# mbrymer/quadrotor_landing

Hardware: NVIDIA B200
Metric: EKF filter-steps/s (propagate+update) (higher is better)
Workload: dtype f64

## Files before the change

### quadrotor_landing_b200/csrc/ekf_kernels.cuh

```cuda
#pragma once

#include <type_traits>

#include "ekf_core.cuh"
#include "ekf_synth.cuh"

namespace qekf {

enum : int32_t {
    FLAG_INIT = 1,
    FLAG_READY = 2,
    FLAG_CORRECTED = 4,
    FLAG_ACTIVE = 8
};

constexpr int AUX_DIM = 11;
constexpr int PEND_DIM = 8;

template <typename T> struct DeviceState {
    T *x;
    T *P;
    T *aux;
    double *pend;
    int32_t *flags;
// ... 27 lines not shown
        return ParUS<T>{ (uint32_t)__cvta_generic_to_shared(csm) };
    }
#endif
};
template <typename T> struct ParSel<T, true> {
    using type = ParF<T>;
    static QEKF_FN type make(const Consts<T> &c, const DeviceState<T> &st, int64_t i)
    {
        return type{ c, st.pf + i, st.pf_delay + i, st.ld };
    }
    static QEKF_FN type make_cold(const type &par, const Consts<T> *, const DeviceState<T> &, int64_t, std::false_type) { return par; }
#ifdef __CUDACC__
    static __device__ __forceinline__ ParFS<T> make_cold(const type &, const Consts<T> *csm, const DeviceState<T> &st, int64_t i, std::true_type)
    {
        return ParFS<T>{ (uint32_t)__cvta_generic_to_shared(csm), st.pf + i, st.pf_delay + i, st.ld };
    }
#endif
};

struct StreamView {
    const double *imu;
    const int32_t *tag_step;
    const double *tag_pose;
    const double *tag_stamp;
    const uint8_t *tag_valid;
    const double *tag_sigma;
    int64_t cs, is;
    int64_t M;
    int64_t vs;
    double t_start;
    double update_freq;
};

template <typename T> struct RunArgs {
    DeviceState<T> st;
    StreamView in;
    Consts<T> c;
    int64_t k0, n_steps;
    int32_t m0;
    NoiseSpec ns;
    StatsView stats;
};

#ifdef __CUDA_ARCH__
#define QEKF_COLD __device__ __noinline__
#else
#define QEKF_COLD inline
#endif

template <typename T, bool SYNTH> struct Inputs {
    const double *imu_i, *tag_i;
    int64_t cs;
    const uint8_t *valid_i;
    int64_t vs;
    int64_t gid;
    double bias[6];
    int32_t priv_start;

    QEKF_FN void init(const RunArgs<T> &a, int64_t i) { init(a, i, i); }
    QEKF_FN void init(const RunArgs<T> &a, int64_t i, int64_t id)
    {
        imu_i = a.in.imu + i * a.in.is;
        tag_i = a.in.tag_pose + i * a.in.is;
        cs = a.in.cs;
        valid_i = (!SYNTH && a.in.tag_valid) ? a.in.tag_valid + i : nullptr;
        vs = a.in.vs;
        gid = a.ns.gid0 + id;
        if (SYNTH) {
            true_bias(a.ns, gid, bias);
            priv_start = private_dropout_start(a.ns, gid);
        }
    }
    QEKF_FN void raw_imu(int64_t k, double u[6]) const
    {
#pragma unroll
// ... 144 lines not shown
    T *x = st.x + i;
#pragma unroll
    for (int k = 0; k < 3; ++k) {
        x[(0 + k) * st.ld] = s.r[k];
        x[(3 + k) * st.ld] = s.v[k];
        x[(10 + k) * st.ld] = s.ab[k];
        x[(13 + k) * st.ld] = s.wb[k];
    }
#pragma unroll
    for (int k = 0; k < 4; ++k) x[(6 + k) * st.ld] = s.q[k];
#pragma unroll 8
    for (int e = 0; e < NP; ++e) st.P[e * st.ld + i] = P.el(e);
}

template <typename T, bool BIAS, bool DIRECT, class PS, class PAR>
QEKF_COLD void correction_call(Nominal<T> *sp, PS &P, const T *tag, const PAR par, Observation<T> *obs)
{
    Nominal<T> s = *sp;
    T tg[7];
#pragma unroll
    for (int cc = 0; cc < 7; ++cc) tg[cc] = tag[cc];
    Observation<T> o;
    correction_step<T, BIAS, DIRECT>(s, P, tg, par, o);
    *sp = s;
    *obs = o;
}

struct CtaVote {
    int active, want, fenced, at_fence, lanes;
    bool out_of_patience;
};
constexpr int VOTE_WORDS = 12;

QEKF_FN void cta_vote_init(int *vbuf)
{
#ifdef __CUDA_ARCH__
    if (threadIdx.x < VOTE_WORDS) vbuf[threadIdx.x] = 0;
    __syncthreads();
#else
    (void)vbuf;
#endif
}

QEKF_FN CtaVote cta_vote(int *vbuf, uint32_t iter, bool active, bool want, bool oop, bool fenced, bool at_fence)
{
    CtaVote r;
#ifdef __CUDA_ARCH__
    const unsigned full = 0xffffffffu;
    const unsigned ma = __ballot_sync(full, active), mw = __ballot_sync(full, want), mo = __ballot_sync(full, oop);
    const unsigned mf = __ballot_sync(full, fenced), mt = __ballot_sync(full, at_fence);
    int *v = vbuf + (iter % 3u) * 4;
    if ((threadIdx.x & 31) == 0) {
        atomicAdd(v + 0, __popc(ma) | (__popc(mw) << 16));
        atomicAdd(v + 1, __popc(mf) | (__popc(mt) << 16));
        if (mo) atomicOr(v + 2, 1);
    }
    __syncthreads();
    const int x0 = v[0], x1 = v[1], x2 = v[2];
    if (threadIdx.x == 0) {
        int *z = vbuf + ((iter + 2u) % 3u) * 4;
        z[0] = 0; z[1] = 0; z[2] = 0;
    }
    r.active = x0 & 0xffff; r.want = x0 >> 16; r.fenced = x1 & 0xffff; r.at_fence = x1 >> 16;
    r.out_of_patience = x2 != 0;
    r.lanes = (int)blockDim.x;
#else
    (void)vbuf; (void)iter;
    r.active = active; r.want = want; r.fenced = fenced; r.at_fence = at_fence; r.out_of_patience = oop; r.lanes = 1;
#endif
    return r;
}

struct WarpVote {
    int active, want, fenced, at_fence, lanes;
    bool out_of_patience;
};
QEKF_FN WarpVote warp_vote(bool active, bool want, bool oop, bool fenced, bool at_fence)
{
    WarpVote r;
#ifdef __CUDA_ARCH__
    const unsigned full = 0xffffffffu;
    r.active = __popc(__ballot_sync(full, active));
    r.want = __popc(__ballot_sync(full, want));
    r.fenced = __popc(__ballot_sync(full, fenced));
    r.at_fence = __popc(__ballot_sync(full, at_fence));
    r.out_of_patience = __ballot_sync(full, oop) != 0u;
    r.lanes = 32;
#else
    r.active = active; r.want = want; r.fenced = fenced; r.at_fence = at_fence; r.out_of_patience = oop; r.lanes = 1;
#endif
    return r;
}
QEKF_FN bool cta_any(bool x)
{
#ifdef __CUDA_ARCH__
    return __syncthreads_or(x) != 0;
#else
    return x;
#endif
}

struct SmemInt {
    int32_t *p;
    QEKF_FN operator int32_t() const { return *p; }
    QEKF_FN SmemInt &operator=(int32_t v) { *p = v; return *this; }
    QEKF_FN SmemInt &operator=(const SmemInt &o) { *p = *o.p; return *this; }
    QEKF_FN SmemInt &operator+=(int32_t v) { *p += v; return *this; }
    QEKF_FN SmemInt &operator-=(int32_t v) { *p -= v; return *this; }
    QEKF_FN SmemInt &operator|=(int32_t v) { *p |= v; return *this; }
    QEKF_FN SmemInt &operator&=(int32_t v) { *p &= v; return *this; }
    QEKF_FN SmemInt &operator++() { *p += 1; return *this; }
};
constexpr int MR_SCRATCH_INTS = 18;
constexpr int SR_SCRATCH_INTS = 16;

template <typename T, bool BIAS, bool DIRECT, bool SYNTH, bool PF, class PS, bool CSM = false>
QEKF_FN void run_filter(const RunArgs<T> &a, const int64_t i_in, PS &P, int32_t *scr, const int scr_stride,
                        const bool live = true, int *vbuf = nullptr, const Consts<T> *c_cold = nullptr)
{
    const Consts<T> &c = a.c;
    const int64_t i = live ? i_in : 0;
    const typename ParSel<T, PF>::type par = ParSel<T, PF>::make(a.c, a.st, i);
    const auto par_cold = ParSel<T, PF>::make_cold(par, c_cold, a.st, i, std::integral_constant<bool, CSM>());
    const int32_t k_end = (int32_t)(a.k0 + a.n_steps);
    Nominal<T> s;
    SmemInt flags{ scr + 0 * scr_stride }, upds{ scr + 1 * scr_stride }, n_pred{ scr + 2 * scr_stride };
    SmemInt n_corr{ scr + 3 * scr_stride }, n_iter{ scr + 4 * scr_stride }, m{ scr + 5 * scr_stride };
    SmemInt next_tag_step{ scr + 6 * scr_stride }, pend_m{ scr + 7 * scr_stride }, held{ scr + 8 * scr_stride };
    SmemInt k{ scr + 9 * scr_stride };
    flags = 0; upds = 0; n_pred = 0; n_corr = 0; n_iter = 0;
    T accel[3] = { T(0), T(0), T(0) };
    Inputs<T, SYNTH> in;
    double un[6] = { 0, 0, 0, 0, 0, 0 };
    k = k_end;
    if (live) {
        load_filter<T>(a.st, i, s, P);
        flags = a.st.flags[i];
        upds = a.st.upds[i];
#pragma unroll
        for (int cc = 0; cc < 3; ++cc) accel[cc] = a.st.aux[cc * a.st.ld + i];
        in.init(a, i, a.st.gid_perm ? (int64_t)a.st.gid_perm[i] : i);
        k = (int32_t)a.k0;
        if (SYNTH) {
            float z[6];
            normals6(a.ns, in.gid, STREAM_BIAS, 0u, z);
#pragma unroll
            for (int cc = 0; cc < 6; ++cc) reinterpret_cast<float *>(scr)[(10 + cc) * scr_stride] = z[cc];
        } else {
            in.raw_imu(k, un);
        }
    }
    auto true_bias_now = [&](double b[6]) {
#pragma unroll
        for (int cc = 0; cc < 6; ++cc)
            b[cc] = (double)(cc < 3 ? a.ns.sig_ba : a.ns.sig_bw) * (double)reinterpret_cast<const float *>(scr)[(10 + cc) * scr_stride];
    };

    uint32_t n_sexec = 0, n_cev = 0;
    m = a.m0;
    next_tag_step = (m < a.in.M) ? a.in.tag_step[m] : INT32_MAX;
    pend_m = -1;
    held = 0;
    bool at_fence = false;
    const bool do_stats = SYNTH && a.stats.acc != nullptr;
    const int32_t patience = c.limit_measurement_freq ? (c.upd_per_meas - 1) : 0;
    int32_t next_fence = do_stats ? (int32_t)((a.k0 / a.stats.stride + 1) * a.stats.stride) : INT32_MAX;
    bool predicted = false;

    cta_vote_init(vbuf);
    for (uint32_t iter = 0;; ++iter) {
        bool want = predicted;
        if (k < k_end && !at_fence && !predicted) {
            int32_t kk = k, up = upds, fl = flags, nts = next_tag_step, np_run = 0;
            for (;;) {
                if (kk == nts) {
                    const int32_t mm = m;
                    if (in.valid(a.in, a.ns, mm, kk)) {
                        pend_m = mm;
                        fl |= FLAG_READY;
                        if (!(fl & FLAG_INIT)) {
                            T tag0[7];
                            in.tag(a.in, a.ns, mm, tag0);
                            initialize_state<T, BIAS>(s, P, tag0, par, false);
                            fl |= FLAG_INIT;
                        }
                    }
                    m = mm + 1;
                    nts = (mm + 1 < a.in.M) ? a.in.tag_step[mm + 1] : INT32_MAX;
                }
                const bool init = (fl & FLAG_INIT) != 0;
                const bool gate = init && (fl & FLAG_READY) && (!c.limit_measurement_freq || (up + 1) >= c.upd_per_meas);
                if (init) {
                    T u[6];
                    if (SYNTH) {
                        double raw[6], tb[6], ud[6];
                        in.raw_imu(a.in, kk, raw);
                        true_bias_now(tb);
                        synth_imu(a.ns, in.gid, kk, raw, tb, ud);
#pragma unroll
                        for (int cc = 0; cc < 6; ++cc) u[cc] = (T)ud[cc];
                    } else {
                        in.imu(a.ns, kk, un, u);
                    }
                    prediction_step<T, BIAS>(s, P, u, par, accel);
                    ++np_run;
                }
                if (gate) { want = true; break; }
                if (init) {
                    up += 1;
                    fl = (fl & ~FLAG_CORRECTED) | FLAG_ACTIVE;
                }
                ++kk;
                if (!SYNTH && kk < k_end) in.raw_imu(kk, un);
                if (kk == next_fence) { at_fence = true; break; }
                if (kk >= k_end) break;
            }
            k = kk; upds = up; flags = fl; next_tag_step = nts;
            n_pred += np_run;
            predicted = want;
        }
        const bool active = (k < k_end) && !at_fence;
        const int32_t fl0 = flags;
        const CtaVote v = cta_vote(vbuf, iter, active, want, want && held >= patience, at_fence || k >= k_end, at_fence);
        if (v.active == 0 && v.at_fence == 0) break;
        ++n_iter;
        if (do_stats && v.fenced == v.lanes && v.at_fence != 0) {
            const bool mine = live && at_fence && (fl0 & FLAG_INIT);
            double tb[6] = { 0, 0, 0, 0, 0, 0 };
            if (SYNTH) true_bias_now(tb);
            stats_sample<T, BIAS>(a, i, (int64_t)k - 1, s, P, tb, mine);
            if (mine) ++n_sexec;
            at_fence = false;
            next_fence += a.stats.stride;
        }
        bool serve = true;
        if (v.want != 0) serve = (2 * v.want > v.active) || v.out_of_patience;
        if (want && !serve) ++held;

#if defined(__CUDA_ARCH__) && defined(QEKF_DIAG_EVENTS)
        if (__ballot_sync(0xffffffffu, want && serve) != 0u) ++n_cev;
#endif
        if (want && serve) {
            T tag[7];
            if (pend_m >= 0) {
                in.tag(a.in, a.ns, pend_m, tag);
            } else {
#pragma unroll
                for (int cc = 0; cc < 7; ++cc) tag[cc] = (T)a.st.pend[cc * a.st.ld + i];
            }
            flags &= ~FLAG_READY;
            const bool perform = c.corner_margin_enbl ? corner_gate<T>(tag, c) : true;
            held = 0;
            if (perform) {
                ++n_corr;
                Observation<T> obs;
                correction_step<T, BIAS, DIRECT>(s, P, tag, par, obs);
// ... 559 lines not shown
        advance(&s, k - nh, nh, accel, a.st.ring + i);
        store_filter<T>(a.st, i, s, P);
        hp = (nh > 0) ? nh - 1 : 0;
    }
    a.st.flags[i] = flags;
    a.st.upds[i] = upds;
    a.st.nh[i] = nh; a.st.hpos[i] = hp; a.st.hlen[i] = hlen;
    if (a.st.counts) {
#ifdef __CUDA_ARCH__
        atomicAdd(a.st.counts + 0, (unsigned long long)(uint32_t)(int32_t)n_pred);
        atomicAdd(a.st.counts + 1, (unsigned long long)n_corr);
        if ((i & 31) == 0) atomicAdd(a.st.counts + 2, (unsigned long long)n_iter);
        atomicAdd(a.st.counts + 4, (unsigned long long)n_sexec);
#else
        a.st.counts[0] += (uint32_t)(int32_t)n_pred;
        a.st.counts[1] += n_corr;
#endif
    }
#pragma unroll
    for (int cc = 0; cc < 3; ++cc) a.st.aux[cc * a.st.ld + i] = accel[cc];
}

template <typename T> __device__ __forceinline__ void copy_consts(Consts<T> *dst, const Consts<T> &src)
{
#ifdef __CUDA_ARCH__
    static_assert(sizeof(Consts<T>) % 8 == 0, "Consts is copied in 8-byte words");
    const unsigned long long *s = reinterpret_cast<const unsigned long long *>(&src);
    unsigned long long *d = reinterpret_cast<unsigned long long *>(dst);
    for (unsigned w = threadIdx.x; w < sizeof(Consts<T>) / 8; w += blockDim.x) d[w] = s[w];
#endif
}
constexpr size_t consts_smem_bytes(size_t consts_size) { return (consts_size + 15) / 16 * 16; }

template <typename T, bool BIAS, bool DIRECT, bool SYNTH, bool MR, bool PF, int BLOCK>
__global__ void __launch_bounds__(BLOCK, 1) run_kernel(const __grid_constant__ RunArgs<T> a)
{
    constexpr int N = BIAS ? 15 : 9;
    extern __shared__ __align__(16) unsigned char smem_raw[];
    T *sm = reinterpret_cast<T *>(smem_raw);
    const int64_t slot = (int64_t)blockIdx.x * BLOCK + threadIdx.x;
    const bool live = slot < a.st.n;
    const int64_t i = slot;
    PShared<T, N, BLOCK> P{ sm + threadIdx.x };
#ifdef QEKF_EXP8
    int *vbuf = reinterpret_cast<int *>(sm + (size_t)BLOCK * ((sizeof(T) == 8 && N == 15) ? 105 : N * (N + 1) / 2));
#else
    int *vbuf = reinterpret_cast<int *>(sm + (size_t)BLOCK * (N * (N + 1) / 2));
#endif
    int32_t *scr = vbuf + VOTE_WORDS;
    Consts<T> *csm = reinterpret_cast<Consts<T> *>(scr + (size_t)BLOCK * (MR ? MR_SCRATCH_INTS : SR_SCRATCH_INTS));
#ifndef QEKF_EXP8
    copy_consts(csm, a.c);
#else
    csm = nullptr;
#endif
#ifndef QEKF_EXP8
    if constexpr (MR && SYNTH) {
        if (a.st.hist_synth) run_filter_mrs<T, BIAS, DIRECT, PF, PShared<T, N, BLOCK>, true>(a, i, P, scr + threadIdx.x, BLOCK, live, vbuf, csm);
        else run_filter_mr<T, BIAS, DIRECT, SYNTH, PF, PShared<T, N, BLOCK>, true>(a, i, P, scr + threadIdx.x, BLOCK, live, vbuf, csm);
    } else if constexpr (MR) {
        run_filter_mr<T, BIAS, DIRECT, SYNTH, PF, PShared<T, N, BLOCK>, true>(a, i, P, scr + threadIdx.x, BLOCK, live, vbuf, csm);
    } else {
        run_filter<T, BIAS, DIRECT, SYNTH, PF, PShared<T, N, BLOCK>, true>(a, i, P, scr + threadIdx.x, BLOCK, live, vbuf, csm);
    }
#else
    if (MR) run_filter_mr<T, BIAS, DIRECT, SYNTH, PF>(a, i, P, scr + threadIdx.x, BLOCK, live, vbuf, csm);
    else run_filter<T, BIAS, DIRECT, SYNTH, PF>(a, i, P, scr + threadIdx.x, BLOCK, live, vbuf, csm);
#endif
}

template <typename T, class PS>
QEKF_FN void rebase_history(const DeviceState<T> &st, int64_t i, const Nominal<T> &s, const PS &P)
{
    if (!st.xc) return;
    store_checkpoint<T>(st, i, s, P);
    st.nh[i] = 0;
    st.hlen[i] = 1;
}

template <typename T, bool BIAS, bool PF, class PS>
QEKF_FN void deliver_one(const DeviceState<T> &st, const Consts<T> &c, const double *pose8, int force_init, int reinit_bias,
                         int raise_ready, PS &P, int64_t i)
{
    int32_t flags = st.flags[i];
    if (!force_init) {
#pragma unroll
        for (int cc = 0; cc < PEND_DIM; ++cc) st.pend[cc * st.ld + i] = pose8[cc];
        if (raise_ready) flags |= FLAG_READY;
    }
    if (force_init || (raise_ready && !(flags & FLAG_INIT))) {
        Nominal<T> s;
        load_filter<T>(st, i, s, P);
        T tag[7];
#pragma unroll
        for (int cc = 0; cc < 7; ++cc) tag[cc] = (T)st.pend[cc * st.ld + i];
        const typename ParSel<T, PF>::type par = ParSel<T, PF>::make(c, st, i);
        initialize_state<T, BIAS>(s, P, tag, par, reinit_bias != 0);
        store_filter<T>(st, i, s, P);
        rebase_history<T>(st, i, s, P);
        flags |= FLAG_INIT;
    }
// ... 132 lines not shown
```

### quadrotor_landing_b200/csrc/ekf_synth.cuh

```cuda
#pragma once

#include <cmath>

#include "ekf_core.cuh"

namespace qekf {

struct NoiseSpec {
    uint64_t seed;
    int64_t gid0;
    float sig_a, sig_w;
    float sig_ba, sig_bw;
    float sig_p, sig_th;
    int32_t drop_k0, drop_k1;
    int32_t rdrop_len, rdrop_lo, rdrop_hi;
    int32_t edge_loss;
    double range_ref, range_exp_p, range_exp_th;
};

enum : uint32_t { STREAM_IMU = 0, STREAM_TAG = 2, STREAM_BIAS = 4, STREAM_DROPOUT = 6 };

QEKF_FN uint32_t mulhi32(uint32_t a, uint32_t b)
{
#ifdef __CUDA_ARCH__
// ... 66 lines not shown

QEKF_FN void true_bias(const NoiseSpec &ns, int64_t gid, double b[6])
{
    float z[6];
    normals6(ns, gid, STREAM_BIAS, 0u, z);
#pragma unroll
    for (int i = 0; i < 3; ++i) {
        b[i] = (double)ns.sig_ba * (double)z[i];
        b[3 + i] = (double)ns.sig_bw * (double)z[3 + i];
    }
}

QEKF_FN int32_t private_dropout_start(const NoiseSpec &ns, int64_t gid)
{
    if (ns.rdrop_len <= 0 || ns.rdrop_hi <= ns.rdrop_lo) return INT32_MAX;
    uint32_t w[4];
    philox4x32_10(0u, STREAM_DROPOUT, (uint32_t)(uint64_t)gid, (uint32_t)((uint64_t)gid >> 32), (uint32_t)ns.seed,
                  (uint32_t)(ns.seed >> 32), w);
    const uint32_t span = (uint32_t)(ns.rdrop_hi - ns.rdrop_lo);
    return ns.rdrop_lo + (int32_t)mulhi32(w[0], span);
}

QEKF_FN bool arrival_valid(const NoiseSpec &ns, int32_t step, int32_t priv_start)
{
    if (step >= ns.drop_k0 && step < ns.drop_k1) return false;
    if (priv_start != INT32_MAX && step >= priv_start && step < priv_start + ns.rdrop_len) return false;
    return true;
}

struct ImuSynth {
    uint64_t seed;
    float sig_a, sig_w, sig_ba, sig_bw;
};
QEKF_FN void synth_imu(const ImuSynth &nz, int64_t gid, int64_t k, const double clean[6], const double bias[6], double u[6])
{
    float z[6];
    normals6(nz.seed, gid, STREAM_IMU, (uint32_t)k, z);
#pragma unroll
    for (int i = 0; i < 3; ++i) {
        u[i] = clean[i] + bias[i] + (double)nz.sig_a * (double)z[i];
        u[3 + i] = clean[3 + i] + bias[3 + i] + (double)nz.sig_w * (double)z[3 + i];
    }
}
QEKF_FN void synth_imu(const NoiseSpec &ns, int64_t gid, int64_t k, const double clean[6], const double bias[6], double u[6])
{
    const ImuSynth nz{ ns.seed, ns.sig_a, ns.sig_w, ns.sig_ba, ns.sig_bw };
    synth_imu(nz, gid, k, clean, bias, u);
}

template <typename T> QEKF_FN bool bundle_in_image(const double tag[7], const Consts<T> &c)
{
    double R[9];
    quat_to_rot<double>(tag + 3, R);
    for (int i = 0; i < c.n_tags; ++i) {
        const double hw = (double)c.tag_hw[i], px0 = (double)c.tag_px[i], py0 = (double)c.tag_py[i];
        bool all_in = true;
#pragma unroll
        for (int k = 0; k < 4; ++k) {
            const double cx = ((k == 0 || k == 3) ? hw : -hw) + px0;
            const double cy = ((k < 2) ? hw : -hw) + py0;
            const double p0 = R[0] * cx + R[1] * cy + tag[0];
            const double p1 = R[3] * cx + R[4] * cy + tag[1];
            const double p2 = R[6] * cx + R[7] * cy + tag[2];
            const double iz = 1.0 / p2;
            const double xn = p0 * iz, yn = p1 * iz;
            const double uu = (double)c.Kcam[0] * xn + (double)c.Kcam[1] * yn + (double)c.Kcam[2];
            const double vv = (double)c.Kcam[3] * xn + (double)c.Kcam[4] * yn + (double)c.Kcam[5];
            all_in = all_in && (p2 > 0.0) && (uu > 0.0) && (uu < (double)c.cam_w) && (vv > 0.0) && (vv < (double)c.cam_h);
        }
        if (all_in) return true;
    }
    return false;
}

inline void visibility_mask(const double *tag_pose_clean, int64_t M, const Consts<double> &c, uint8_t *out)
// ... 122 lines not shown
```

### quadrotor_landing_b200/csrc/inst_run.cu

```cuda
#include "launch.hpp"

namespace qekf {

template <typename T, bool BIAS, bool DIRECT, bool SYNTH, bool MR, bool PF>
cudaError_t launch_run(const RunArgs<T> &a, unsigned grid, size_t smem, cudaStream_t stream)
{
    auto kern = run_kernel<T, BIAS, DIRECT, SYNTH, MR, PF, BlockOf<T>::value>;
    cudaError_t e = prep_kernel(kern, smem);
    if (e != cudaSuccess) return e;
    kern<<<grid, BlockOf<T>::value, smem, stream>>>(a);
    return cudaGetLastError();
}

template <typename T, bool BIAS, bool DIRECT, bool MR>
cudaError_t launch_tick(const RunArgs<T> &a, const double *pose8, int tag_mode, double *out, int n_out, cudaStream_t stream)
{
    constexpr int N = BIAS ? 15 : 9;
    auto kern = tick_kernel<T, BIAS, DIRECT, MR>;
    const size_t smem = (size_t)TICK_BLOCK * (N * (N + 1) / 2) * sizeof(T) + VOTE_WORDS * sizeof(int) +
                        (size_t)TICK_BLOCK * (MR ? MR_SCRATCH_INTS : SR_SCRATCH_INTS) * sizeof(int32_t);
    static unsigned prepared = 0;
    int dev = 0;
    cudaGetDevice(&dev);
    if (!(prepared & (1u << (dev & 31)))) {
        cudaError_t e = cudaFuncSetAttribute(kern, cudaFuncAttributeMaxDynamicSharedMemorySize, (int)smem);
        if (e != cudaSuccess) return e;
        prepared |= 1u << (dev & 31);
    }
    const unsigned grid = (unsigned)((a.st.n + TICK_BLOCK - 1) / TICK_BLOCK);
    kern<<<grid, TICK_BLOCK, smem, stream>>>(a, pose8, tag_mode, out, n_out);
    return cudaGetLastError();
}
template cudaError_t launch_tick<Q_T, (Q_BIAS != 0), (Q_DIRECT != 0), (Q_MR != 0)>(const RunArgs<Q_T> &, const double *, int,
                                                                                   double *, int, cudaStream_t);

#define INST(S, PF_)                                                                                                  \
    template cudaError_t launch_run<Q_T, (Q_BIAS != 0), (Q_DIRECT != 0), S, (Q_MR != 0), PF_>(const RunArgs<Q_T> &,    \
                                                                                               unsigned, size_t, cudaStream_t);
INST(false, false)
INST(true, false)
INST(false, true)
INST(true, true)

// ... 2 lines not shown
```

### quadrotor_landing_b200/csrc/launch.hpp

```cpp
#pragma once

#include <cuda_runtime.h>

#include "ekf_kernels.cuh"

namespace qekf {

#ifdef QEKF_EXP8
template <typename T> struct BlockOf { static constexpr int value = (sizeof(T) == 4) ? 384 : 256; };
#else
#ifndef QEKF_FP32_BLOCK
#define QEKF_FP32_BLOCK 384
#endif
template <typename T> struct BlockOf { static constexpr int value = (sizeof(T) == 4) ? QEKF_FP32_BLOCK : 224; };
#endif

template <typename T, bool BIAS, bool DIRECT, bool SYNTH, bool MR, bool PF>
cudaError_t launch_run(const RunArgs<T> &a, unsigned grid, size_t smem, cudaStream_t stream);

template <typename T, bool BIAS, bool PF>
cudaError_t launch_deliver(const DeviceState<T> &st, const Consts<T> &c, const double *pose8, int force_init,
                           int reinit_bias, int raise_ready, unsigned grid, size_t smem, cudaStream_t stream);

template <typename T, bool BIAS, bool DIRECT, bool MR>
cudaError_t launch_tick(const RunArgs<T> &a, const double *pose8, int tag_mode, double *out, int n_out, cudaStream_t stream);

template <typename T, bool BIAS, bool PF>
cudaError_t launch_predict(const DeviceState<T> &st, const Consts<T> &c, const double *u, unsigned grid, size_t smem,
                           cudaStream_t stream);

template <typename T, bool BIAS, bool DIRECT, bool PF>
cudaError_t launch_correct(const DeviceState<T> &st, const Consts<T> &c, const double *tag, unsigned grid, size_t smem,
                           cudaStream_t stream);

template <typename T>
cudaError_t launch_reset(const DeviceState<T> &st, const Consts<T> &c, int nstates, int reset_nominal, cudaStream_t stream);

template <typename T> cudaError_t launch_rebase(const DeviceState<T> &st, int np, cudaStream_t stream);

template <typename T>
cudaError_t launch_dump(const RunArgs<T> &a, int64_t first, int64_t count, int64_t T_ticks, double *imu_out,
                        double *tag_out, uint8_t *valid_out, double *bias_out, cudaStream_t stream);

template <typename W>
cudaError_t launch_permute_rows(W *dst, const W *src, const int32_t *perm, int64_t rows, int64_t ld, int64_t n, bool to_slots,
                                cudaStream_t stream);

template <typename T> cudaError_t launch_fma_peak(T *sink, int iters, unsigned grid, unsigned block, cudaStream_t stream);
// ... 12 lines not shown
```

### quadrotor_landing_b200/csrc/qekf_capi.cu

```cuda
#include "../../include/qekf.h"

#include <cuda_runtime.h>

#include <algorithm>
#include <cmath>
#include <cstdio>
#include <cstdlib>
#include <cstring>
#include <new>
#include <string>
#include <type_traits>
#include <vector>

#include "ekf_params.hpp"
#include "launch.hpp"
#include "launch_coop.hpp"
#include "preset.hpp"
#include "scenario.hpp"

using namespace qekf;

namespace {

thread_local std::string g_err;
// ... 26 lines not shown
    double *pend = nullptr;
    int32_t *flags = nullptr, *upds = nullptr;
    unsigned long long *counts = nullptr;
    void *xc = nullptr, *Pc = nullptr, *ring = nullptr;
    int32_t *nh = nullptr, *hpos = nullptr, *hlen = nullptr;
    int ring_len = 0, dmax = 1;
    std::vector<double> pf_host[5];
    bool pf_overridden[5] = { false, false, false, false, false };
    bool pf_on = false;
    void *pf = nullptr;
    double *pf_delay = nullptr;
    double *d_tick = nullptr;
    double *h_tick = nullptr;
    double *tick_in = nullptr, *tick_in_dev = nullptr;
    double *tick_out = nullptr, *tick_out_dev = nullptr;
    int tick_out_cap = 0;
    int32_t *d_no_steps = nullptr;
    double imu_latched[6] = { 0, 0, 0, 0, 0, 0 };
    void *d_in = nullptr;
    size_t d_in_bytes = 0;
    double *stats_acc = nullptr, *stats_red = nullptr;
    int32_t stats_bins = 0, stats_stride = 0;
    void *d_shared = nullptr;
    size_t d_shared_bytes = 0;
    uint8_t *d_mask = nullptr;
    size_t d_mask_bytes = 0;
    int32_t *d_perm = nullptr;
    void *perm_scratch = nullptr;
    size_t perm_scratch_bytes = 0;
    bool in_slot_order = false;
    uint64_t perm_seed = 0;
    int64_t perm_gid0 = 0;
    int32_t perm_len = 0, perm_lo = 0, perm_hi = 0;
    bool perm_on = true;
    int64_t perm_min_steps = 256;
    bool hist_clean = true, hist_key_valid = false, lazy_mr_on = true, lazy_now = false;
    uint64_t hist_key[6] = { 0, 0, 0, 0, 0, 0 };
    int64_t hist_k_next = 0;
    int64_t launches = 0;
    int lanes_per_filter = 1;
    int coop_groups = COOP_GROUPS_DEFAULT, duo_groups = DUO_GROUPS_DEFAULT;
};

namespace {

template <typename T> DeviceState<T> dstate(const qekf_handle *h)
{
    DeviceState<T> s;
    s.x = (T *)h->x; s.P = (T *)h->P; s.aux = (T *)h->aux; s.pend = h->pend;
    s.flags = h->flags; s.upds = h->upds; s.counts = h->counts; s.ld = h->ld; s.n = h->n;
    s.xc = (T *)h->xc; s.Pc = (T *)h->Pc; s.ring = (T *)h->ring;
    s.nh = h->nh; s.hpos = h->hpos; s.hlen = h->hlen;
    s.ring_len = h->ring_len; s.dmax_m1 = h->dmax - 1;
    s.pf = h->pf_on ? (const T *)h->pf : nullptr;
    s.pf_delay = h->pf_on ? h->pf_delay : nullptr;
    s.perm = nullptr;
    s.gid_perm = nullptr;
    s.hist_synth = 0;
    return s;
}

void hist_touch(qekf_handle *h) { h->hist_clean = false; h->hist_key_valid = false; }
void hist_emptied(qekf_handle *h) { h->hist_clean = true; h->hist_key_valid = false; }

uint64_t fnv1a(const void *data, size_t bytes, uint64_t hsh = 1469598103934665603ULL)
{
    const unsigned char *p = static_cast<const unsigned char *>(data);
    for (size_t i = 0; i < bytes; ++i) { hsh ^= p[i]; hsh *= 1099511628211ULL; }
    return hsh;
}

int block_of(const qekf_handle *h) { return h->precision == QEKF_FP64 ? BlockOf<double>::value : BlockOf<float>::value; }
size_t smem_bytes(const qekf_handle *h)
{
#ifdef QEKF_EXP8
    size_t b = (size_t)block_of(h) * ((h->precision == QEKF_FP64 && h->np == 120) ? 105 : h->np) * h->tsize + VOTE_WORDS * sizeof(int);
#else
    size_t b = (size_t)block_of(h) * h->np * h->tsize + VOTE_WORDS * sizeof(int);
#endif
    b += (size_t)block_of(h) * (h->p.multirate_ekf ? MR_SCRATCH_INTS : SR_SCRATCH_INTS) * sizeof(int32_t);
#ifndef QEKF_EXP8
    b += consts_smem_bytes(h->precision == QEKF_FP64 ? sizeof(Consts<double>) : sizeof(Consts<float>));
#endif
    return b;
}
unsigned grid_of(const qekf_handle *h) { return (unsigned)((h->n + block_of(h) - 1) / block_of(h)); }

#define QEKF_DISPATCH(h, CALL)                                                             \
    do {                                                                                   \
        const bool b__ = (h)->p.est_bias != 0, d__ = (h)->p.direct_orien_method != 0;      \
        if ((h)->precision == QEKF_FP64) {                                                 \
            if (b__ && d__) { CALL(double, true, true); }                                  \
            else if (b__) { CALL(double, true, false); }                                   \
            else if (d__) { CALL(double, false, true); }                                   \
            else { CALL(double, false, false); }                                           \
        } else {                                                                           \
            if (b__ && d__) { CALL(float, true, true); }                                   \
            else if (b__) { CALL(float, true, false); }                                    \
            else if (d__) { CALL(float, false, true); }                                    \
            else { CALL(float, false, false); }                                            \
        }                                                                                  \
    } while (0)

int free_state(qekf_handle *h)
{
    cudaFree(h->x); cudaFree(h->P); cudaFree(h->aux); cudaFree(h->pend);
    cudaFree(h->flags); cudaFree(h->upds); cudaFree(h->d_tick); cudaFree(h->d_in);
    cudaFree(h->stats_acc); cudaFree(h->stats_red); cudaFree(h->d_shared); cudaFree(h->counts);
    cudaFree(h->xc); cudaFree(h->Pc); cudaFree(h->ring); cudaFree(h->nh); cudaFree(h->hpos); cudaFree(h->hlen);
    cudaFree(h->pf); cudaFree(h->pf_delay); cudaFree(h->d_mask); cudaFree(h->d_perm); cudaFree(h->perm_scratch);
    h->d_perm = nullptr; h->perm_len = 0; h->perm_scratch = nullptr; h->perm_scratch_bytes = 0; h->in_slot_order = false;
    h->d_mask = nullptr; h->d_mask_bytes = 0;
    h->xc = h->Pc = h->ring = nullptr; h->nh = h->hpos = h->hlen = nullptr; h->ring_len = 0;
    h->pf = nullptr; h->pf_delay = nullptr; h->pf_on = false;
    for (auto &v : h->pf_host) v.clear();
    h->counts = nullptr;
    h->stats_acc = h->stats_red = nullptr; h->stats_bins = 0; h->d_shared = nullptr; h->d_shared_bytes = 0;
    if (h->h_tick) cudaFreeHost(h->h_tick);
    if (h->tick_in) cudaFreeHost(h->tick_in);
    if (h->tick_out) cudaFreeHost(h->tick_out);
    h->tick_in = h->tick_in_dev = h->tick_out = h->tick_out_dev = nullptr; h->tick_out_cap = 0;
    h->x = h->P = h->aux = nullptr; h->pend = nullptr; h->flags = h->upds = nullptr;
    h->d_tick = nullptr; h->h_tick = nullptr; h->d_in = nullptr; h->d_in_bytes = 0;
    return QEKF_OK;
}

int max_step_delay(const qekf_handle *h)
{
    if (h->p.dynamic_meas_delay) return step_of_delay(h->p.measurement_delay_max, h->p.update_freq);
    int d = step_of_delay(h->p.measurement_delay, h->p.update_freq);
    const std::vector<double> &v = h->pf_host[QEKF_PF_DELAY];
    for (int64_t i = 0; i < (int64_t)v.size() / 2; ++i) {
        const int di = step_of_delay(v[(size_t)i], h->p.update_freq);
        if (di > d) d = di;
    }
    return d;
}

int alloc_history(qekf_handle *h)
{
    if (!h->p.multirate_ekf) return QEKF_OK;
    const size_t ld = (size_t)h->ld;
    const int dmax = max_step_delay(h);
// ... 32 lines not shown
}

int alloc_state(qekf_handle *h)
{
    h->nstates = h->p.est_bias ? 15 : 9;
    h->np = h->nstates * (h->nstates + 1) / 2;
    h->tsize = (h->precision == QEKF_FP64) ? 8 : 4;
    const size_t ld = (size_t)h->ld;
    CUDA_TRY(cudaMalloc(&h->x, 16 * ld * h->tsize));
    CUDA_TRY(cudaMalloc(&h->P, (size_t)h->np * ld * h->tsize));
    CUDA_TRY(cudaMalloc(&h->aux, AUX_DIM * ld * h->tsize));
    CUDA_TRY(cudaMalloc(&h->pend, PEND_DIM * ld * sizeof(double)));
    CUDA_TRY(cudaMalloc(&h->flags, ld * sizeof(int32_t)));
    CUDA_TRY(cudaMalloc(&h->upds, ld * sizeof(int32_t)));
    CUDA_TRY(cudaMalloc(&h->counts, 8 * sizeof(unsigned long long)));
    CUDA_TRY(cudaMemsetAsync(h->counts, 0, 8 * sizeof(unsigned long long), h->stream));
    CUDA_TRY(cudaMalloc(&h->d_tick, 16 * sizeof(double)));
    CUDA_TRY(cudaMallocHost(&h->h_tick, 16 * sizeof(double)));
    CUDA_TRY(cudaMemsetAsync(h->x, 0, 16 * ld * h->tsize, h->stream));
    CUDA_TRY(cudaMemsetAsync(h->P, 0, (size_t)h->np * ld * h->tsize, h->stream));
    CUDA_TRY(cudaMemsetAsync(h->aux, 0, AUX_DIM * ld * h->tsize, h->stream));
    CUDA_TRY(cudaMemsetAsync(h->pend, 0, PEND_DIM * ld * sizeof(double), h->stream));
    CUDA_TRY(cudaMemsetAsync(h->flags, 0, ld * sizeof(int32_t), h->stream));
    CUDA_TRY(cudaMemsetAsync(h->upds, 0, ld * sizeof(int32_t), h->stream));
    return alloc_history(h);
}

int reset_cov(qekf_handle *h, bool reset_nominal)
{
    if (h->precision == QEKF_FP64)
        CUDA_TRY(launch_reset<double>(dstate<double>(h), make_consts<double>(h->p), h->nstates, reset_nominal, h->stream));
    else
        CUDA_TRY(launch_reset<float>(dstate<float>(h), make_consts<float>(h->p), h->nstates, reset_nominal, h->stream));
    return QEKF_OK;
}

int check_params(const qekf_params *p)
{
    if (!p) return fail(QEKF_ERR_BAD_ARG, "params is NULL");
    if (!(p->update_freq > 0) || !(p->measurement_freq > 0)) return fail(QEKF_ERR_BAD_ARG, "rates must be positive");
    if (p->n_tags < 0 || p->n_tags > QEKF_MAX_TAGS) return fail(QEKF_ERR_BAD_ARG, "n_tags out of range");
    if (p->multirate_ekf) {
        if (!(p->measurement_delay_max >= 0) || !(p->measurement_delay >= 0))
            return fail(QEKF_ERR_BAD_ARG, "measurement delays must be non-negative");
        if (step_of_delay(p->dynamic_meas_delay ? p->measurement_delay_max : p->measurement_delay, p->update_freq) > 4096)
            return fail(QEKF_ERR_BAD_ARG, "measurement delay spans more than 4096 ticks");
    }
    return QEKF_OK;
}

template <typename T, bool BIAS, bool DIRECT>
int run_typed(qekf_handle *h, const StreamView &in, int64_t k0, int64_t n_steps, int32_t m0, const NoiseSpec *ns,
              const double *truth)
{
    RunArgs<T> a;
    std::memset(&a, 0, sizeof a);
    a.st = dstate<T>(h);
    a.in = in;
    a.c = make_consts<T>(h->p);
    a.k0 = k0; a.n_steps = n_steps; a.m0 = m0;
    if (ns) {
        a.ns = *ns;
        a.st.gid_perm = h->in_slot_order ? h->d_perm : nullptr;
        a.st.hist_synth = h->lazy_now ? 1 : 0;
        if (h->stats_acc && truth && h->stats_stride > 0) {
            a.stats.acc = h->stats_acc; a.stats.truth = truth;
            a.stats.n_bins = h->stats_bins; a.stats.stride = h->stats_stride;
            a.stats.chi2_lo = BIAS ? 6.262137795043251 : 2.7003894999803584;
            a.stats.chi2_hi = BIAS ? 27.488392863442982 : 19.02276779864163;
        }
    }
    const bool mr = h->p.multirate_ekf != 0, pf = h->pf_on;
    if constexpr (std::is_same<T, double>::value) {
        if (!mr && h->lanes_per_filter == 2) {
            cudaError_t e;
            if (ns) e = pf ? launch_run_duo<BIAS, DIRECT, true, true>(a, h->duo_groups, h->stream)
                           : launch_run_duo<BIAS, DIRECT, true, false>(a, h->duo_groups, h->stream);
            else e = pf ? launch_run_duo<BIAS, DIRECT, false, true>(a, h->duo_groups, h->stream)
                        : launch_run_duo<BIAS, DIRECT, false, false>(a, h->duo_groups, h->stream);
            if (e != cudaSuccess) return fail(QEKF_ERR_CUDA, std::string("two-role replay launch: ") + cudaGetErrorString(e));
            h->launches++;
            return QEKF_OK;
        }
        if (!mr && h->lanes_per_filter == 3) {
            cudaError_t e;
            if (ns) e = pf ? launch_run_coop<BIAS, DIRECT, true, true>(a, h->coop_groups, h->stream)
                           : launch_run_coop<BIAS, DIRECT, true, false>(a, h->coop_groups, h->stream);
            else e = pf ? launch_run_coop<BIAS, DIRECT, false, true>(a, h->coop_groups, h->stream)
                        : launch_run_coop<BIAS, DIRECT, false, false>(a, h->coop_groups, h->stream);
            if (e != cudaSuccess) return fail(QEKF_ERR_CUDA, std::string("cooperative replay launch: ") + cudaGetErrorString(e));
            h->launches++;
            return QEKF_OK;
        }
    }
#define LAUNCH_(S, MR_, PF_) CUDA_TRY((launch_run<T, BIAS, DIRECT, S, MR_, PF_>(a, grid_of(h), smem_bytes(h), h->stream)))
#define LAUNCH_S(S)                                                       \
    do {                                                                  \
        if (mr && pf) LAUNCH_(S, true, true);                             \
        else if (mr) LAUNCH_(S, true, false);                             \
        else if (pf) LAUNCH_(S, false, true);                             \
        else LAUNCH_(S, false, false);                                    \
    } while (0)
    if (ns) LAUNCH_S(true);
    else LAUNCH_S(false);
#undef LAUNCH_S
#undef LAUNCH_
    h->launches++;
    return QEKF_OK;
}

int run_dispatch(qekf_handle *h, const StreamView &in, int64_t k0, int64_t n_steps, int32_t m0,
                 const NoiseSpec *ns = nullptr, const double *truth = nullptr)
{
#define CALL_RUN(T, B, D) return run_typed<T, B, D>(h, in, k0, n_steps, m0, ns, truth)
    QEKF_DISPATCH(h, CALL_RUN);
#undef CALL_RUN
    return QEKF_OK;
}

int fetch_rows(qekf_handle *h, const void *dev, int rows, int64_t first, int64_t count, double *out)
{
    CUDA_TRY(cudaStreamSynchronize(h->stream));
    if (h->precision == QEKF_FP64) {
        CUDA_TRY(cudaMemcpy2D(out, (size_t)count * 8, (const char *)dev + (size_t)first * 8, (size_t)h->ld * 8,
                              (size_t)count * 8, (size_t)rows, cudaMemcpyDeviceToHost));
    } else {
        std::vector<float> tmp((size_t)rows * (size_t)count);
        CUDA_TRY(cudaMemcpy2D(tmp.data(), (size_t)count * 4, (const char *)dev + (size_t)first * 4, (size_t)h->ld * 4,
// ... 1206 lines not shown
```

Before: 8.102 billion.

## Add producer warp that precomputes IMU noise into a per-block shared ring

For fp64 Monte-Carlo single-rate runs, the kernel gains an extra warp that generates Gaussian IMU noise ahead of the filter threads. It writes the noise into a global slab ring claimed per block and publishes progress with release/acquire flags in shared memory. Filter threads spin-wait on those flags, read the precomputed noise, and prefetch the next tick's noise and IMU data. Vote barriers switch to a named barrier that covers only the filter threads. The goal is to take RNG cost off the filter's critical path, at the cost of extra threads, spin-waiting, global-memory ring traffic and slab-claim atomics.

```diff
diff --git a/quadrotor_landing_b200/csrc/ekf_kernels.cuh b/quadrotor_landing_b200/csrc/ekf_kernels.cuh
--- a/quadrotor_landing_b200/csrc/ekf_kernels.cuh
+++ b/quadrotor_landing_b200/csrc/ekf_kernels.cuh
@@ -83,6 +83,14 @@
     double update_freq;
 };
 
+struct NoiseRing {
+    float *slab;
+    int32_t *owner;
+    int32_t n_slabs;
+};
+constexpr int NOISE_RING_TICKS = 16;
+constexpr int NOISE_BATCH = 4;
+
 template <typename T> struct RunArgs {
     DeviceState<T> st;
     StreamView in;
@@ -91,7 +99,17 @@
     int32_t m0;
     NoiseSpec ns;
     StatsView stats;
+    NoiseRing nring;
 };
+
+template <typename T, bool SYNTH, bool MR> QEKF_FN constexpr bool has_noise_producer()
+{
+#ifdef QEKF_EXP8
+    return false;
+#else
+    return sizeof(T) == 8 && SYNTH && !MR;
+#endif
+}
 
 #ifdef __CUDA_ARCH__
 #define QEKF_COLD __device__ __noinline__
@@ -302,16 +320,25 @@
 };
 constexpr int VOTE_WORDS = 12;
 
-QEKF_FN void cta_vote_init(int *vbuf)
+template <int NT> QEKF_FN void filter_sync()
+{
+#ifdef __CUDA_ARCH__
+    if constexpr (NT == 0) __syncthreads();
+    else asm volatile("bar.sync 1, %0;" ::"n"(NT) : "memory");
+#endif
+}
+
+template <int NT = 0> QEKF_FN void cta_vote_init(int *vbuf)
 {
 #ifdef __CUDA_ARCH__
     if (threadIdx.x < VOTE_WORDS) vbuf[threadIdx.x] = 0;
-    __syncthreads();
+    filter_sync<NT>();
 #else
     (void)vbuf;
 #endif
 }
 
+template <int NT = 0>
 QEKF_FN CtaVote cta_vote(int *vbuf, uint32_t iter, bool active, bool want, bool oop, bool fenced, bool at_fence)
 {
     CtaVote r;
@@ -325,7 +352,7 @@
         atomicAdd(v + 1, __popc(mf) | (__popc(mt) << 16));
         if (mo) atomicOr(v + 2, 1);
     }
-    __syncthreads();
+    filter_sync<NT>();
     const int x0 = v[0], x1 = v[1], x2 = v[2];
     if (threadIdx.x == 0) {
         int *z = vbuf + ((iter + 2u) % 3u) * 4;
@@ -333,7 +360,7 @@
     }
     r.active = x0 & 0xffff; r.want = x0 >> 16; r.fenced = x1 & 0xffff; r.at_fence = x1 >> 16;
     r.out_of_patience = x2 != 0;
-    r.lanes = (int)blockDim.x;
+    r.lanes = NT ? NT : (int)blockDim.x;
 #else
     (void)vbuf; (void)iter;
     r.active = active; r.want = want; r.fenced = fenced; r.at_fence = at_fence; r.out_of_patience = oop; r.lanes = 1;
@@ -383,11 +410,60 @@
 };
 constexpr int MR_SCRATCH_INTS = 18;
 constexpr int SR_SCRATCH_INTS = 16;
-
-template <typename T, bool BIAS, bool DIRECT, bool SYNTH, bool PF, class PS, bool CSM = false>
+constexpr int SR_K_WORD = 9;
+QEKF_FN constexpr int noise_prod_smem_ints(int rows) { return rows + 4; }
+
+QEKF_FN int32_t ld_acquire_cta(const int32_t *p)
+{
+#ifdef __CUDA_ARCH__
+    int32_t v;
+    asm volatile("ld.acquire.cta.shared.b32 %0, [%1];" : "=r"(v) : "r"((uint32_t)__cvta_generic_to_shared(p)) : "memory");
+    return v;
+#else
+    return *p;
+#endif
+}
+QEKF_FN int32_t ld_relaxed_cta(const int32_t *p)
+{
+#ifdef __CUDA_ARCH__
+    int32_t v;
+    asm volatile("ld.relaxed.cta.shared.b32 %0, [%1];" : "=r"(v) : "r"((uint32_t)__cvta_generic_to_shared(p)) : "memory");
+    return v;
+#else
+    return *p;
+#endif
+}
+QEKF_FN void st_release_cta(int32_t *p, int32_t v)
+{
+#ifdef __CUDA_ARCH__
+    asm volatile("st.release.cta.shared.b32 [%0], %1;" ::"r"((uint32_t)__cvta_generic_to_shared(p)), "r"(v) : "memory");
+#else
+    *p = v;
+#endif
+}
+QEKF_FN void st_relaxed_cta(int32_t *p, int32_t v)
+{
+#ifdef __CUDA_ARCH__
+    asm volatile("st.relaxed.cta.shared.b32 [%0], %1;" ::"r"((uint32_t)__cvta_generic_to_shared(p)), "r"(v) : "memory");
+#else
+    *p = v;
+#endif
+}
+template <typename T> QEKF_FN void prefetch_l1(const T *p)
+{
+#ifdef __CUDA_ARCH__
+    asm volatile("prefetch.global.L1 [%0];" ::"l"(p));
+#else
+    (void)p;
+#endif
+}
+
+template <typename T, bool BIAS, bool DIRECT, bool SYNTH, bool PF, class PS, bool CSM = false, int NT = 0>
 QEKF_FN void run_filter(const RunArgs<T> &a, const int64_t i_in, PS &P, int32_t *scr, const int scr_stride,
-                        const bool live = true, int *vbuf = nullptr, const Consts<T> *c_cold = nullptr)
-{
+                        const bool live = true, int *vbuf = nullptr, const Consts<T> *c_cold = nullptr,
+                        const float *zring = nullptr, const int32_t *zprod = nullptr)
+{
+    static_assert(NT == 0 || SYNTH, "only Monte-Carlo launches have a noise producer");
     const Consts<T> &c = a.c;
     const int64_t i = live ? i_in : 0;
     const typename ParSel<T, PF>::type par = ParSel<T, PF>::make(a.c, a.st, i);
@@ -397,12 +473,12 @@
     SmemInt flags{ scr + 0 * scr_stride }, upds{ scr + 1 * scr_stride }, n_pred{ scr + 2 * scr_stride };
     SmemInt n_corr{ scr + 3 * scr_stride }, n_iter{ scr + 4 * scr_stride }, m{ scr + 5 * scr_stride };
     SmemInt next_tag_step{ scr + 6 * scr_stride }, pend_m{ scr + 7 * scr_stride }, held{ scr + 8 * scr_stride };
-    SmemInt k{ scr + 9 * scr_stride };
+    SmemInt k{ scr + SR_K_WORD * scr_stride };
     flags = 0; upds = 0; n_pred = 0; n_corr = 0; n_iter = 0;
     T accel[3] = { T(0), T(0), T(0) };
     Inputs<T, SYNTH> in;
     double un[6] = { 0, 0, 0, 0, 0, 0 };
-    k = k_end;
+    k = live ? (int32_t)a.k0 : k_end;
     if (live) {
         load_filter<T>(a.st, i, s, P);
         flags = a.st.flags[i];
@@ -410,7 +486,6 @@
 #pragma unroll
         for (int cc = 0; cc < 3; ++cc) accel[cc] = a.st.aux[cc * a.st.ld + i];
         in.init(a, i, a.st.gid_perm ? (int64_t)a.st.gid_perm[i] : i);
-        k = (int32_t)a.k0;
         if (SYNTH) {
             float z[6];
             normals6(a.ns, in.gid, STREAM_BIAS, 0u, z);
@@ -437,7 +512,7 @@
     int32_t next_fence = do_stats ? (int32_t)((a.k0 / a.stats.stride + 1) * a.stats.stride) : INT32_MAX;
     bool predicted = false;
 
-    cta_vote_init(vbuf);
+    cta_vote_init<NT>(vbuf);
     for (uint32_t iter = 0;; ++iter) {
         bool want = predicted;
         if (k < k_end && !at_fence && !predicted) {
@@ -466,7 +541,29 @@
                         double raw[6], tb[6], ud[6];
                         in.raw_imu(a.in, kk, raw);
                         true_bias_now(tb);
-                        synth_imu(a.ns, in.gid, kk, raw, tb, ud);
+                        if constexpr (NT > 0) {
+                            if (ld_acquire_cta(zprod) <= kk) {
+                                while (ld_acquire_cta(zprod) <= kk) {
+#ifdef __CUDA_ARCH__
+                                    __nanosleep(64);
+#endif
+                                }
+                            }
+                            float z[6];
+                            const float *e = zring + (kk & (NOISE_RING_TICKS - 1)) * 6 * NT;
+#pragma unroll
+                            for (int cc = 0; cc < 6; ++cc) z[cc] = e[cc * NT];
+                            if (kk + 1 < k_end) {
+                                const float *e1 = zring + ((kk + 1) & (NOISE_RING_TICKS - 1)) * 6 * NT;
+#pragma unroll
+                                for (int cc = 0; cc < 6; ++cc) prefetch_l1(e1 + cc * NT);
+                                prefetch_l1(a.in.imu + (int64_t)(kk + 1) * 6);
+                                prefetch_l1(a.in.imu + (int64_t)(kk + 1) * 6 + 5);
+                            }
+                            apply_imu_noise(a.ns.sig_a, a.ns.sig_w, z, raw, tb, ud);
+                        } else {
+                            synth_imu(a.ns, in.gid, kk, raw, tb, ud);
+                        }
 #pragma unroll
                         for (int cc = 0; cc < 6; ++cc) u[cc] = (T)ud[cc];
                     } else {
@@ -481,6 +578,7 @@
                     fl = (fl & ~FLAG_CORRECTED) | FLAG_ACTIVE;
                 }
                 ++kk;
+                if constexpr (NT > 0) st_relaxed_cta(k.p, kk);
                 if (!SYNTH && kk < k_end) in.raw_imu(kk, un);
                 if (kk == next_fence) { at_fence = true; break; }
                 if (kk >= k_end) break;
@@ -491,7 +589,7 @@
         }
         const bool active = (k < k_end) && !at_fence;
         const int32_t fl0 = flags;
-        const CtaVote v = cta_vote(vbuf, iter, active, want, want && held >= patience, at_fence || k >= k_end, at_fence);
+        const CtaVote v = cta_vote<NT>(vbuf, iter, active, want, want && held >= patience, at_fence || k >= k_end, at_fence);
         if (v.active == 0 && v.at_fence == 0) break;
         ++n_iter;
         if (do_stats && v.fenced == v.lanes && v.at_fence != 0) {
@@ -1117,14 +1215,62 @@
 }
 constexpr size_t consts_smem_bytes(size_t consts_size) { return (consts_size + 15) / 16 * 16; }
 
+#ifdef __CUDACC__
+template <typename T, int NT>
+__device__ void noise_producer(const RunArgs<T> &a, float *slab, int32_t *prod, const int32_t *kword)
+{
+    const unsigned full = 0xffffffffu;
+    const int32_t k_end = (int32_t)(a.k0 + a.n_steps);
+    const int64_t row0 = (int64_t)blockIdx.x * NT;
+    for (;;) {
+        bool done = true, idle = true;
+        for (int j = (int)(threadIdx.x & 31); j < NT; j += 32) {
+            const int32_t p = prod[j];
+            if (p >= k_end) continue;
+            done = false;
+            const int32_t lim = min(min(ld_relaxed_cta(kword + j) + NOISE_RING_TICKS, k_end), p + NOISE_BATCH);
+            if (lim <= p) continue;
+            idle = false;
+            const int64_t row = row0 + j;
+            const int64_t gid = a.ns.gid0 + (a.st.gid_perm ? (int64_t)a.st.gid_perm[row] : row);
+            for (int32_t t = p; t < lim; ++t) {
+                float z[6];
+                normals6(a.ns, gid, STREAM_IMU, (uint32_t)t, z);
+                float *e = slab + (t & (NOISE_RING_TICKS - 1)) * 6 * NT + j;
+#pragma unroll
+                for (int cc = 0; cc < 6; ++cc) e[cc * NT] = z[cc];
+            }
+            st_release_cta(prod + j, lim);
+        }
+        if (__all_sync(full, done)) return;
+        if (__all_sync(full, idle)) __nanosleep(256);
+    }
+}
+
+__device__ __forceinline__ int32_t claim_noise_slab(const NoiseRing &r)
+{
+    int32_t s = (int32_t)(blockIdx.x % (unsigned)r.n_slabs);
+    while (atomicCAS(r.owner + s, 0, 1) != 0) s = (s + 1 == r.n_slabs) ? 0 : s + 1;
+    __threadfence();
+    return s;
+}
+__device__ __forceinline__ void release_noise_slab(const NoiseRing &r, int32_t s)
+{
+    __threadfence();
+    atomicExch(r.owner + s, 0);
+}
+#endif
+
 template <typename T, bool BIAS, bool DIRECT, bool SYNTH, bool MR, bool PF, int BLOCK>
-__global__ void __launch_bounds__(BLOCK, 1) run_kernel(const __grid_constant__ RunArgs<T> a)
+__global__ void __launch_bounds__(BLOCK + (has_noise_producer<T, SYNTH, MR>() ? 32 : 0), 1)
+run_kernel(const __grid_constant__ RunArgs<T> a)
 {
     constexpr int N = BIAS ? 15 : 9;
+    constexpr bool PROD = has_noise_producer<T, SYNTH, MR>();
     extern __shared__ __align__(16) unsigned char smem_raw[];
     T *sm = reinterpret_cast<T *>(smem_raw);
     const int64_t slot = (int64_t)blockIdx.x * BLOCK + threadIdx.x;
-    const bool live = slot < a.st.n;
+    const bool live = threadIdx.x < BLOCK && slot < a.st.n;
     const int64_t i = slot;
     PShared<T, N, BLOCK> P{ sm + threadIdx.x };
 #ifdef QEKF_EXP8
@@ -1133,25 +1279,46 @@
     int *vbuf = reinterpret_cast<int *>(sm + (size_t)BLOCK * (N * (N + 1) / 2));
 #endif
     int32_t *scr = vbuf + VOTE_WORDS;
-    Consts<T> *csm = reinterpret_cast<Consts<T> *>(scr + (size_t)BLOCK * (MR ? MR_SCRATCH_INTS : SR_SCRATCH_INTS));
+    int32_t *prod = scr + (size_t)BLOCK * (MR ? MR_SCRATCH_INTS : SR_SCRATCH_INTS);
+    Consts<T> *csm = reinterpret_cast<Consts<T> *>(prod + (PROD ? noise_prod_smem_ints(BLOCK) : 0));
 #ifndef QEKF_EXP8
     copy_consts(csm, a.c);
 #else
     csm = nullptr;
 #endif
+    if constexpr (PROD) {
+        int32_t *slab_idx = prod + BLOCK;
+        if (threadIdx.x == 0) *slab_idx = claim_noise_slab(a.nring);
+        const int32_t k_end = (int32_t)(a.k0 + a.n_steps);
+        if (threadIdx.x < BLOCK) {
+            const int32_t k_first = live ? (int32_t)a.k0 : k_end;
+            scr[SR_K_WORD * BLOCK + threadIdx.x] = k_first;
+            prod[threadIdx.x] = k_first;
+        }
+        __syncthreads();
+        float *slab = a.nring.slab + (size_t)*slab_idx * (NOISE_RING_TICKS * 6 * BLOCK);
+        if (threadIdx.x >= BLOCK)
+            noise_producer<T, BLOCK>(a, slab, prod, scr + SR_K_WORD * BLOCK);
+        else
+            run_filter<T, BIAS, DIRECT, SYNTH, PF, PShared<T, N, BLOCK>, true, BLOCK>(a, i, P, scr + threadIdx.x, BLOCK, live, vbuf,
+                                                                                    csm, slab + threadIdx.x, prod + threadIdx.x);
+        __syncthreads();
+        if (threadIdx.x == 0) release_noise_slab(a.nring, *slab_idx);
+    } else {
 #ifndef QEKF_EXP8
-    if constexpr (MR && SYNTH) {
-        if (a.st.hist_synth) run_filter_mrs<T, BIAS, DIRECT, PF, PShared<T, N, BLOCK>, true>(a, i, P, scr + threadIdx.x, BLOCK, live, vbuf, csm);
-        else run_filter_mr<T, BIAS, DIRECT, SYNTH, PF, PShared<T, N, BLOCK>, true>(a, i, P, scr + threadIdx.x, BLOCK, live, vbuf, csm);
-    } else if constexpr (MR) {
-        run_filter_mr<T, BIAS, DIRECT, SYNTH, PF, PShared<T, N, BLOCK>, true>(a, i, P, scr + threadIdx.x, BLOCK, live, vbuf, csm);
-    } else {
-        run_filter<T, BIAS, DIRECT, SYNTH, PF, PShared<T, N, BLOCK>, true>(a, i, P, scr + threadIdx.x, BLOCK, live, vbuf, csm);
-    }
-#else
-    if (MR) run_filter_mr<T, BIAS, DIRECT, SYNTH, PF>(a, i, P, scr + threadIdx.x, BLOCK, live, vbuf, csm);
-    else run_filter<T, BIAS, DIRECT, SYNTH, PF>(a, i, P, scr + threadIdx.x, BLOCK, live, vbuf, csm);
-#endif
+        if constexpr (MR && SYNTH) {
+            if (a.st.hist_synth) run_filter_mrs<T, BIAS, DIRECT, PF, PShared<T, N, BLOCK>, true>(a, i, P, scr + threadIdx.x, BLOCK, live, vbuf, csm);
+            else run_filter_mr<T, BIAS, DIRECT, SYNTH, PF, PShared<T, N, BLOCK>, true>(a, i, P, scr + threadIdx.x, BLOCK, live, vbuf, csm);
+        } else if constexpr (MR) {
+            run_filter_mr<T, BIAS, DIRECT, SYNTH, PF, PShared<T, N, BLOCK>, true>(a, i, P, scr + threadIdx.x, BLOCK, live, vbuf, csm);
+        } else {
+            run_filter<T, BIAS, DIRECT, SYNTH, PF, PShared<T, N, BLOCK>, true>(a, i, P, scr + threadIdx.x, BLOCK, live, vbuf, csm);
+        }
+#else
+        if (MR) run_filter_mr<T, BIAS, DIRECT, SYNTH, PF>(a, i, P, scr + threadIdx.x, BLOCK, live, vbuf, csm);
+        else run_filter<T, BIAS, DIRECT, SYNTH, PF>(a, i, P, scr + threadIdx.x, BLOCK, live, vbuf, csm);
+#endif
+    }
 }
 
 template <typename T, class PS>
diff --git a/quadrotor_landing_b200/csrc/ekf_synth.cuh b/quadrotor_landing_b200/csrc/ekf_synth.cuh
--- a/quadrotor_landing_b200/csrc/ekf_synth.cuh
+++ b/quadrotor_landing_b200/csrc/ekf_synth.cuh
@@ -122,15 +122,19 @@
     uint64_t seed;
     float sig_a, sig_w, sig_ba, sig_bw;
 };
+QEKF_FN void apply_imu_noise(float sig_a, float sig_w, const float z[6], const double clean[6], const double bias[6], double u[6])
+{
+#pragma unroll
+    for (int i = 0; i < 3; ++i) {
+        u[i] = clean[i] + bias[i] + (double)sig_a * (double)z[i];
+        u[3 + i] = clean[3 + i] + bias[3 + i] + (double)sig_w * (double)z[3 + i];
+    }
+}
 QEKF_FN void synth_imu(const ImuSynth &nz, int64_t gid, int64_t k, const double clean[6], const double bias[6], double u[6])
 {
     float z[6];
     normals6(nz.seed, gid, STREAM_IMU, (uint32_t)k, z);
-#pragma unroll
-    for (int i = 0; i < 3; ++i) {
-        u[i] = clean[i] + bias[i] + (double)nz.sig_a * (double)z[i];
-        u[3 + i] = clean[3 + i] + bias[3 + i] + (double)nz.sig_w * (double)z[3 + i];
-    }
+    apply_imu_noise(nz.sig_a, nz.sig_w, z, clean, bias, u);
 }
 QEKF_FN void synth_imu(const NoiseSpec &ns, int64_t gid, int64_t k, const double clean[6], const double bias[6], double u[6])
 {
diff --git a/quadrotor_landing_b200/csrc/inst_run.cu b/quadrotor_landing_b200/csrc/inst_run.cu
--- a/quadrotor_landing_b200/csrc/inst_run.cu
+++ b/quadrotor_landing_b200/csrc/inst_run.cu
@@ -8,7 +8,7 @@
     auto kern = run_kernel<T, BIAS, DIRECT, SYNTH, MR, PF, BlockOf<T>::value>;
     cudaError_t e = prep_kernel(kern, smem);
     if (e != cudaSuccess) return e;
-    kern<<<grid, BlockOf<T>::value, smem, stream>>>(a);
+    kern<<<grid, run_threads<T, SYNTH, MR>(), smem, stream>>>(a);
     return cudaGetLastError();
 }
 
diff --git a/quadrotor_landing_b200/csrc/launch.hpp b/quadrotor_landing_b200/csrc/launch.hpp
--- a/quadrotor_landing_b200/csrc/launch.hpp
+++ b/quadrotor_landing_b200/csrc/launch.hpp
@@ -14,6 +14,10 @@
 #endif
 template <typename T> struct BlockOf { static constexpr int value = (sizeof(T) == 4) ? QEKF_FP32_BLOCK : 224; };
 #endif
+template <typename T, bool SYNTH, bool MR> constexpr int run_threads()
+{
+    return BlockOf<T>::value + (has_noise_producer<T, SYNTH, MR>() ? 32 : 0);
+}
 
 template <typename T, bool BIAS, bool DIRECT, bool SYNTH, bool MR, bool PF>
 cudaError_t launch_run(const RunArgs<T> &a, unsigned grid, size_t smem, cudaStream_t stream);
diff --git a/quadrotor_landing_b200/csrc/qekf_capi.cu b/quadrotor_landing_b200/csrc/qekf_capi.cu
--- a/quadrotor_landing_b200/csrc/qekf_capi.cu
+++ b/quadrotor_landing_b200/csrc/qekf_capi.cu
@@ -82,6 +82,9 @@
     uint64_t perm_seed = 0;
     int64_t perm_gid0 = 0;
     int32_t perm_len = 0, perm_lo = 0, perm_hi = 0;
+    float *nring_slab = nullptr;
+    int32_t *nring_owner = nullptr;
+    int32_t nring_slabs = 0;
     bool perm_on = true;
     int64_t perm_min_steps = 256;
     bool hist_clean = true, hist_key_valid = false, lazy_mr_on = true, lazy_now = false;
@@ -121,7 +124,7 @@
 }
 
 int block_of(const qekf_handle *h) { return h->precision == QEKF_FP64 ? BlockOf<double>::value : BlockOf<float>::value; }
-size_t smem_bytes(const qekf_handle *h)
+size_t smem_bytes(const qekf_handle *h, bool synth = false)
 {
 #ifdef QEKF_EXP8
     size_t b = (size_t)block_of(h) * ((h->precision == QEKF_FP64 && h->np == 120) ? 105 : h->np) * h->tsize + VOTE_WORDS * sizeof(int);
@@ -129,6 +132,8 @@
     size_t b = (size_t)block_of(h) * h->np * h->tsize + VOTE_WORDS * sizeof(int);
 #endif
     b += (size_t)block_of(h) * (h->p.multirate_ekf ? MR_SCRATCH_INTS : SR_SCRATCH_INTS) * sizeof(int32_t);
+    if (h->precision == QEKF_FP64 ? has_noise_producer<double, true, false>() : has_noise_producer<float, true, false>())
+        if (synth && !h->p.multirate_ekf) b += (size_t)noise_prod_smem_ints(block_of(h)) * sizeof(int32_t);
 #ifndef QEKF_EXP8
     b += consts_smem_bytes(h->precision == QEKF_FP64 ? sizeof(Consts<double>) : sizeof(Consts<float>));
 #endif
@@ -159,6 +164,8 @@
     cudaFree(h->stats_acc); cudaFree(h->stats_red); cudaFree(h->d_shared); cudaFree(h->counts);
     cudaFree(h->xc); cudaFree(h->Pc); cudaFree(h->ring); cudaFree(h->nh); cudaFree(h->hpos); cudaFree(h->hlen);
     cudaFree(h->pf); cudaFree(h->pf_delay); cudaFree(h->d_mask); cudaFree(h->d_perm); cudaFree(h->perm_scratch);
+    cudaFree(h->nring_slab); cudaFree(h->nring_owner);
+    h->nring_slab = nullptr; h->nring_owner = nullptr; h->nring_slabs = 0;
     h->d_perm = nullptr; h->perm_len = 0; h->perm_scratch = nullptr; h->perm_scratch_bytes = 0; h->in_slot_order = false;
     h->d_mask = nullptr; h->d_mask_bytes = 0;
     h->xc = h->Pc = h->ring = nullptr; h->nh = h->hpos = h->hlen = nullptr; h->ring_len = 0;
@@ -257,6 +264,18 @@
         CUDA_TRY(launch_reset<double>(dstate<double>(h), make_consts<double>(h->p), h->nstates, reset_nominal, h->stream));
     else
         CUDA_TRY(launch_reset<float>(dstate<float>(h), make_consts<float>(h->p), h->nstates, reset_nominal, h->stream));
+    return QEKF_OK;
+}
+
+int ensure_noise_ring(qekf_handle *h)
+{
+    if (h->nring_slab) return QEKF_OK;
+    int sms = 0;
+    CUDA_TRY(cudaDeviceGetAttribute(&sms, cudaDevAttrMultiProcessorCount, h->device));
+    CUDA_TRY(cudaMalloc(&h->nring_slab, (size_t)sms * NOISE_RING_TICKS * 6 * BlockOf<double>::value * sizeof(float)));
+    CUDA_TRY(cudaMalloc(&h->nring_owner, (size_t)sms * sizeof(int32_t)));
+    CUDA_TRY(cudaMemsetAsync(h->nring_owner, 0, (size_t)sms * sizeof(int32_t), h->stream));
+    h->nring_slabs = sms;
     return QEKF_OK;
 }
 
@@ -318,7 +337,12 @@
             return QEKF_OK;
         }
     }
-#define LAUNCH_(S, MR_, PF_) CUDA_TRY((launch_run<T, BIAS, DIRECT, S, MR_, PF_>(a, grid_of(h), smem_bytes(h), h->stream)))
+    if (ns && !mr && has_noise_producer<T, true, false>()) {
+        const int e = ensure_noise_ring(h);
+        if (e != QEKF_OK) return e;
+        a.nring.slab = h->nring_slab; a.nring.owner = h->nring_owner; a.nring.n_slabs = h->nring_slabs;
+    }
+#define LAUNCH_(S, MR_, PF_) CUDA_TRY((launch_run<T, BIAS, DIRECT, S, MR_, PF_>(a, grid_of(h), smem_bytes(h, S), h->stream)))
 #define LAUNCH_S(S)                                                       \
     do {                                                                  \
         if (mr && pf) LAUNCH_(S, true, true);                             \
```

After: 8.212 billion (median of 6 runs). 1.01x the previous value.
